# 2gunsu/monocon-pytorch

Measured on AMD Instinct MI355X. Metric: images/sec (384x1280) fwd+bwd, higher is better.
Workload: dtype f32 (f16x2); 1 GPU; train step B=32/GPU 3x384x1280 (configs[2] shape, fp32 values, mode f16x2); global_batch=32, parallelism=dp1, precision_mode=f16x2

## Files before the change

### monocon-pytorch_amd/csrc/kernels_head_train.hip

```cpp
#include <type_traits>

#include "kernels.h"
#include "train.h"

namespace mc {

struct HeadBwdArgs {
    const float *draw; int ld;
    const unsigned *nz; int nz_tiles;
    const float *z, *x, *w1;
    const float *scale, *shift;
    float *d, *dw_partial, *red_partial;
    int HW, rows_per_block, blocks_per_img;
    const float *coef;
    float *csum;
    unsigned *amax;
};
constexpr int HB_PX = 64, HB_LD = 80;
static bool head_rows_as_coded() {
    const int *rbeg = head_row_begin();
    static const int RB[NUM_HEADS + 1] = {0, 3, 5, 7, 25, 34, 36, 39, 41, 65};
    for (int i = 0; i <= NUM_HEADS; ++i)
        if (rbeg[i] != RB[i]) return false;
    return true;
}
__device__ __forceinline__ int head_of_row(int r) {
    return (r >= 3) + (r >= 5) + (r >= 7) + (r >= 25) + (r >= 34) + (r >= 36) + (r >= 39) + (r >= 41);
}
constexpr int HB_WAVES = 4, HB_NT = HB_WAVES * 64, HB_MAXR = 24;

template <int RB, int NR, int MODE>
struct HeadPart {
    static constexpr int CP = NUM_HEADS * HEAD_CH;
    float w[NR], acc[NR];
    float s1, s2, zsc, zsh, cp, cq, cr;
    const float *xp, *zp;
    float *dp;
    bool rez;
    int h, sub, nsub;

    __device__ __forceinline__ void init(const HeadBwdArgs &a, int h_, int lane, size_t p0, int b, int sub_, int nsub_) {
        h = h_; sub = sub_; nsub = nsub_;
#pragma unroll
        for (int r = 0; r < NR; ++r) { w[r] = a.w1[(RB + r) * HEAD_CH + lane]; acc[r] = 0.f; }
        s1 = 0.f; s2 = 0.f;
        rez = a.z == nullptr;
        zsc = rez ? a.scale[(size_t)b * CP + h * HEAD_CH + lane] : 0.f;
        zsh = rez ? a.shift[(size_t)b * CP + h * HEAD_CH + lane] : 0.f;
        xp = a.x + p0 * CP + h * HEAD_CH + lane;
// ... 63 lines not shown
        int k = 0;
        for (; k + U <= cnt; k += U) {
            float xv[U];
#pragma unroll
            for (int u = 0; u < U; ++u) xv[u] = xp[(size_t)(px0 + sub + (k + u) * nsub) * CP];
#pragma unroll
            for (int u = 0; u < U; ++u) {
                const float o = fmaf(cq, xv[u], cr);
                s1 += o;
                s2 = fmaxf(s2, fabsf(o));
                dp[(size_t)(px0 + sub + (k + u) * nsub) * CP] = o;
            }
        }
        for (; k < cnt; ++k) {
            const size_t gp = (size_t)(px0 + sub + k * nsub);
            const float o = fmaf(cq, xp[gp * CP], cr);
            s1 += o;
            s2 = fmaxf(s2, fabsf(o));
            dp[gp * CP] = o;
        }
    }
    __device__ __forceinline__ void spill(float *red, int lane) const {
        if (nsub == 1 || sub == 0) return;
        float *q = red + (size_t)(sub - 1) * (NR + 2) * 64 + lane;
        if (MODE != 2) {
#pragma unroll
            for (int r = 0; r < NR; ++r) q[r * 64] = acc[r];
        }
        q[NR * 64] = s1;
        q[(NR + 1) * 64] = s2;
    }
    __device__ __forceinline__ void finish(const HeadBwdArgs &a, const float *red, int blk, int lane) {
        if (MODE == 2 && a.amax) amax_update_wave(a.amax, s2);
        if (sub != 0) return;
        for (int k = 1; k < nsub; ++k) {
            const float *q = red + (size_t)(k - 1) * (NR + 2) * 64 + lane;
            if (MODE != 2) {
#pragma unroll
                for (int r = 0; r < NR; ++r) acc[r] += q[r * 64];
                s2 += q[(NR + 1) * 64];
            }
            s1 += q[NR * 64];
        }
        if (MODE == 2) {
            a.csum[((size_t)blk * CP + h * HEAD_CH + lane) * 2] = s1;
            return;
        }
#pragma unroll
        for (int r = 0; r < NR; ++r) a.dw_partial[((size_t)blk * NUM_OUT_ROWS + RB + r) * HEAD_CH + lane] = acc[r];
        float *rp = a.red_partial + ((size_t)blk * CP + h * HEAD_CH + lane) * 2;
        rp[0] = s1;
        rp[1] = s2;
    }
};

template <int RB, int NR, int MODE>
__device__ __forceinline__ void head_bwd_one(const HeadBwdArgs &a, float *gsh, float *red, int h, int wv, int lane, size_t p0, int np,
                                             int blk, int b, int r0) {
    HeadPart<RB, NR, MODE> P;
    P.init(a, h, lane, p0, b, wv, HB_WAVES);
    const unsigned *nzb = a.nz ? a.nz + (size_t)b * a.nz_tiles : nullptr;
    auto live = [&](int px0) -> bool {
        if (!nzb) return true;
        const int first = r0 + px0, last = r0 + min(px0 + HB_PX, np) - 1;
        const unsigned m = nzb[first >> 6] | nzb[last >> 6];
        return (__builtin_amdgcn_readfirstlane(m) >> h) & 1u;
// ... 15 lines not shown
        const bool nxt = px0 + HB_PX < np && live(px0 + HB_PX);
        if (cur) {
            __syncthreads();
#pragma unroll
            for (int k = 0; k < NL; ++k) {
                const int e = tid + k * HB_NT;
                if (e < NE) gsh[e] = pre[k];
            }
            __syncthreads();
            if (nxt) fetch(px0 + HB_PX);
            P.block(gsh, px0, min(HB_PX, np - px0));
        } else {
            if (nxt) fetch(px0 + HB_PX);
            P.zero_block(px0, min(HB_PX, np - px0));
        }
        cur = nxt;
    }
    P.spill(red, lane);
    __syncthreads();
    P.finish(a, red, blk, lane);
}
template <int MODE, bool WIDE>
__global__ __launch_bounds__(HB_NT) void head_bwd_kernel(const HeadBwdArgs a) {
    __shared__ float gsh[HB_PX * (WIDE ? HB_MAXR : 3)];
    __shared__ float red[(HB_WAVES - 1) * ((WIDE ? HB_MAXR : 3) + 2) * 64];
    const int lane = threadIdx.x & 63;
    const int wv = __builtin_amdgcn_readfirstlane(threadIdx.x >> 6);
    const int blk = blockIdx.x;
    const int b = blk / a.blocks_per_img, rb = blk % a.blocks_per_img;
    const int r0 = rb * a.rows_per_block;
    const int np = min(a.HW, r0 + a.rows_per_block) - r0;
    const size_t p0 = (size_t)b * a.HW + r0;
    if (WIDE) {
        switch (blockIdx.y) {
            case 0: head_bwd_one<41, 24, MODE>(a, gsh, red, 8, wv, lane, p0, np, blk, b, r0); break;
            case 1: head_bwd_one<7, 18, MODE>(a, gsh, red, 3, wv, lane, p0, np, blk, b, r0); break;
            default: head_bwd_one<25, 9, MODE>(a, gsh, red, 4, wv, lane, p0, np, blk, b, r0); break;
        }
    } else {
        switch (blockIdx.y) {
            case 0: head_bwd_one<0, 3, MODE>(a, gsh, red, 0, wv, lane, p0, np, blk, b, r0); break;
            case 1: head_bwd_one<3, 2, MODE>(a, gsh, red, 1, wv, lane, p0, np, blk, b, r0); break;
            case 2: head_bwd_one<5, 2, MODE>(a, gsh, red, 2, wv, lane, p0, np, blk, b, r0); break;
            case 3: head_bwd_one<34, 2, MODE>(a, gsh, red, 5, wv, lane, p0, np, blk, b, r0); break;
            case 4: head_bwd_one<36, 3, MODE>(a, gsh, red, 6, wv, lane, p0, np, blk, b, r0); break;
            default: head_bwd_one<39, 2, MODE>(a, gsh, red, 7, wv, lane, p0, np, blk, b, r0); break;
        }
    }
}
template <int MODE>
static void head_bwd_launch(const HeadBwdArgs &a, int blocks, hipStream_t st) {
    hipLaunchKernelGGL((head_bwd_kernel<MODE, true>), dim3(blocks, 3), dim3(HB_NT), 0, st, a);
    hipLaunchKernelGGL((head_bwd_kernel<MODE, false>), dim3(blocks, 6), dim3(HB_NT), 0, st, a);
}
static hipError_t head_bwd_args(HeadBwdArgs &a, const float *draw, int ld, const float *z, const float *x, const float *w1, int B,
                                int HW, int blocks, const float *scale, const float *shift, const unsigned *nz) {
    if (!head_rows_as_coded()) return hipErrorInvalidValue;
    if (blocks % B || ld != HB_LD) return hipErrorInvalidValue;
    if (!z && (!scale || !shift)) return hipErrorInvalidValue;
    a = HeadBwdArgs{};
    a.draw = draw; a.ld = ld; a.z = z; a.x = x; a.w1 = w1;
    a.scale = scale; a.shift = shift;
    a.nz = nz; a.nz_tiles = (HW + 63) / 64;
    a.HW = HW; a.blocks_per_img = blocks / B; a.rows_per_block = (HW + a.blocks_per_img - 1) / a.blocks_per_img;
    return hipSuccess;
}
hipError_t launch_head_bwd(const float *draw, int ld, const float *z, const float *x, const float *w1, int B, int HW,
                           int blocks, float *d, float *dw_partial, float *red_partial, hipStream_t st, const float *scale,
                           const float *shift, const unsigned *nz) {
    HeadBwdArgs a;
    hipError_t e = head_bwd_args(a, draw, ld, z, x, w1, B, HW, blocks, scale, shift, nz);
    if (e != hipSuccess) return e;
    a.d = d; a.dw_partial = dw_partial; a.red_partial = red_partial;
    if (d) head_bwd_launch<0>(a, blocks, st);
    else head_bwd_launch<1>(a, blocks, st);
    return hipGetLastError();
}
hipError_t launch_head_dx(const float *draw, int ld, const float *x, const float *w1, const float *coef, int B, int HW, int blocks,
                          float *dx, float *csum, float *csum_out, unsigned *amax, hipStream_t st, const float *scale,
                          const float *shift, const unsigned *nz) {
    if (!coef || !dx || !csum || !csum_out) return hipErrorInvalidValue;
    HeadBwdArgs a;
    hipError_t e = head_bwd_args(a, draw, ld, nullptr, x, w1, B, HW, blocks, scale, shift, nz);
    if (e != hipSuccess) return e;
    a.d = dx; a.coef = coef; a.csum = csum; a.amax = amax;
    head_bwd_launch<2>(a, blocks, st);
    return launch_colsum_final(csum, blocks, NUM_HEADS * HEAD_CH, csum_out, st);
}


struct DpredPackArgs {
    const float *dpred[10];
    int ld, B, HW;
    float *out;
    unsigned *nz;
    int row_pred[NUM_OUT_ROWS], row_ch[NUM_OUT_ROWS], pred_c[10];
};
struct DpredUserArgs : DpredPackArgs {
    const float *grad[10];
    const float *pred[10];
    int row_epi[NUM_OUT_ROWS];
};
__device__ __forceinline__ float pred_act_grad(int epi, float y) {
    if (epi == 1) return (y > 1e-4f && y < 1.f - 1e-4f) ? y * (1.f - y) : 0.f;
    if (epi == 2) {
        const float sig = 1.f / (y + 1.f) - 1e-12f;
        return -sig * (1.f - sig) / ((sig + 1e-12f) * (sig + 1e-12f));
    }
    return 1.f;
}
template <bool USER>
__global__ __launch_bounds__(256) void dpred_pack_kernel(const std::conditional_t<USER, DpredUserArgs, DpredPackArgs> a) {
    __shared__ float t[64][NUM_OUT_ROWS + 2];
    __shared__ const float *rowp[NUM_OUT_ROWS];
    __shared__ const float *rowg[USER ? NUM_OUT_ROWS : 1], *rowy[USER ? NUM_OUT_ROWS : 1];
    __shared__ int rowe[USER ? NUM_OUT_ROWS : 1];
    __shared__ unsigned nzw;
    if (threadIdx.x == 0) nzw = 0u;
    const int tiles = (a.HW + 63) / 64;
// ... 637 lines not shown
```

### monocon-pytorch_amd/csrc/mc_train_plan.hip

```cpp
#include <atomic>
#include <deque>
#include <functional>

#include "mc_internal.h"

using namespace mc;

namespace {

using Fn = std::function<int(mc_handle *, hipStream_t)>;

struct PlanSwitches {
    long long lazy_z;
    long long lazy_min;
    long long lazy_feat;
    long long zbits;
    long long grad_pool;
    long long grad_pool_cool;
    long long head_dx_fuse;
    long long head_zskip;
    long long dgrad_s2_thin;
    long long stem_fuse;
    long long bm_epilogue;
    long long wres_bwd;
    long long dual_stream;
    int side_sync_lo = 0, side_sync_hi = 0;
    bool plan_debug = false;
};
const struct { const char *name; long long PlanSwitches::*field; long long def; } SWITCH_TABLE[] = {
    {"MONOCON_HIP_LAZY_Z", &PlanSwitches::lazy_z, 3},
    {"MONOCON_HIP_LAZY_MIN", &PlanSwitches::lazy_min, 900000},
    {"MONOCON_HIP_LAZY_FEAT", &PlanSwitches::lazy_feat, 0},
    {"MONOCON_HIP_ZBITS", &PlanSwitches::zbits, 1},
    {"MONOCON_HIP_GRAD_POOL", &PlanSwitches::grad_pool, 1},
    {"MONOCON_HIP_GRAD_POOL_COOL", &PlanSwitches::grad_pool_cool, 2},
    {"MONOCON_HIP_HEAD_DX_FUSE", &PlanSwitches::head_dx_fuse, 1},
    {"MONOCON_HIP_HEAD_ZSKIP", &PlanSwitches::head_zskip, 1},
    {"MONOCON_HIP_DGRAD_S2_THIN", &PlanSwitches::dgrad_s2_thin, 1},
    {"MONOCON_HIP_STEM_FUSE", &PlanSwitches::stem_fuse, 1},
    {"MONOCON_HIP_BM_EPILOGUE", &PlanSwitches::bm_epilogue, 1},
    {"MONOCON_HIP_WRES_BWD", &PlanSwitches::wres_bwd, 0},
    {"MONOCON_HIP_DUAL_STREAM", &PlanSwitches::dual_stream, 1},
};
PlanSwitches read_switches() {
    PlanSwitches sw{};
    std::string changed;
    for (const auto &d : SWITCH_TABLE) {
        const char *e = std::getenv(d.name);
        sw.*d.field = e ? std::atoll(e) : d.def;
        if (sw.*d.field != d.def) changed += std::string(" ") + d.name + "=" + std::to_string(sw.*d.field);
    }
    if (const char *e = std::getenv("MONOCON_HIP_SIDE_SYNC")) {
        if (std::sscanf(e, "%d:%d", &sw.side_sync_lo, &sw.side_sync_hi) != 2) sw.side_sync_lo = sw.side_sync_hi = 0;
        if (sw.side_sync_lo < sw.side_sync_hi) changed += std::string(" MONOCON_HIP_SIDE_SYNC=") + e;
    }
    sw.plan_debug = std::getenv("MONOCON_HIP_PLAN_DEBUG") != nullptr;
    if (sw.plan_debug && !changed.empty()) fprintf(stderr, "[plan] switches off their defaults:%s\n", changed.c_str());
    return sw;
}

struct PoolBwdArgs {
    const float *x, *dout, *la, *lb;
    float *dx, *stats;
    int B, H, W, C, acc;
};

struct LastWriter {
    enum Kind { NONE, DGRAD_CONV, POOL_BWD, DECONV_BWD } kind = NONE;
    union {
        ConvPlan *conv;
// ... 597 lines not shown
        { size_t o = 0; for (int i = 0; i < 15; ++i) { tp[i] = ta ? ta + o : nullptr; o += up(tn[i]); } }
        T.center_heatmap_target = tp[0]; T.kpt_heatmap_target = tp[1];
        T.wh_target = tp[2]; T.offset_target = tp[3]; T.dim_target = tp[4];
        T.alpha_cls_target = tp[5]; T.alpha_offset_target = tp[6]; T.depth_target = tp[7];
        T.center2kpt_offset_target = tp[8]; T.kpt_heatmap_offset_target = tp[9];
        T.indices = reinterpret_cast<int64_t *>(tp[10]); T.indices_kpt = reinterpret_cast<int64_t *>(tp[11]);
        T.mask_target = reinterpret_cast<uint8_t *>(tp[12]);
        T.mask_center2kpt_offset = tp[13]; T.mask_kpt_heatmap_offset = tp[14];
        h->tgt_arena = ta; h->tgt_arena_bytes = ttot * sizeof(float);
        ts->dpred[0] = alloc((size_t)B * PRED_CH[0] * HW);
        ts->dpred[1] = alloc((size_t)B * PRED_CH[1] * HW);
        size_t dtot = 0;
        for (int i = 2; i < 10; ++i) dtot += up((size_t)B * PRED_CH[i] * HW);
        float *da = alloc(dtot);
        { size_t o = 0; for (int i = 2; i < 10; ++i) { ts->dpred[i] = da ? da + o : nullptr; o += up((size_t)B * PRED_CH[i] * HW); } }
        h->dp_arena = da; h->dp_arena_bytes = dtot * sizeof(float);
        ts->fwd.push_back([ts = ts, B = B, fh = fh, fw = fw](mc_handle *hh, hipStream_t st) {
            if (mc_make_targets(hh, &ts->labels, B, ts->max_objs, ts->pad_h, ts->pad_w, fh, fw, &ts->targets, st)) return -1;
            if (mc_losses(hh, ts->preds, &ts->targets, B, ts->max_objs, fh, fw, ts->losses, st)) return -1;
            return 0;
        });
    }

    void heads_backward(int feat) {
        float *draw = alloc(raw_numel);
        const size_t nz_words = (size_t)B * ((HW + 63) / 64);
        unsigned *nz = sw.head_zskip ? reinterpret_cast<unsigned *>(alloc(nz_words)) : nullptr;
        const unsigned *nz_bwd = nz, *nz_dx = sw.head_zskip == 1 ? nz : nullptr;
        if (sw.plan_debug)
            fprintf(stderr, "[plan] heads backward: zero-tile skip %s (%zu tile words)\n",
                    !sw.head_zskip ? "off" : sw.head_zskip == 1 ? "on" : "on in the statistics pass only", sw.head_zskip ? nz_words : (size_t)0);
        float *cs1 = alloc(colsum_partial_floats((size_t)B * HW, LD));
        float *db1 = alloc(NUM_OUT_ROWS), *dw1 = alloc((size_t)NUM_OUT_ROWS * HEAD_CH);
        push_bwd([=, ts = ts, B = B, fh = fh, fw = fw, HW = HW](mc_handle *hh, hipStream_t st) {
            if (mc_losses_backward(hh, ts->preds, &ts->targets, B, ts->max_objs, fh, fw, ts->grad_losses, ts->dpred, st)) return -1;
            bool user = false;
            for (const float *g : ts->grad_preds) user = user || g != nullptr;
            if (user)
                HIPCHK(hh, launch_dpred_pack_user(ts->dpred, ts->preds, ts->grad_preds, LD, B, HW, draw, st, nz));
            else
                HIPCHK(hh, launch_dpred_pack(ts->dpred, LD, B, HW, draw, st, nz));
            HIPCHK(hh, launch_colsum(draw, (size_t)B * HW, NUM_OUT_ROWS, LD, cs1, db1, st));
            return 0;
        });
        const int nbr = chan_reduce_blocks(B, HW), rb_per_img = nbr / B;
        const bool dx_fuse = sw.head_dx_fuse != 0;
        float *dh = alloc(xh.numel());
        float *dw1p = alloc((size_t)nbr * NUM_OUT_ROWS * HEAD_CH);
        float *partial = alloc((size_t)nbr * CP * 2), *coef = alloc((size_t)B * CP * 4);
        float *dx = dh;
        CopyBatch segcb;
        auto seg = [&](const std::string &layer, int r0, int nr) {
            if (!segcb.add(dw1 + (size_t)r0 * HEAD_CH, G(layer + ".weight", nr * HEAD_CH), (size_t)nr * HEAD_CH) ||
                !segcb.add(db1 + r0, G(layer + ".bias", nr), nr))
                ts->ok = false;
        };
        for (int hd = 0; hd < NUM_HEADS; ++hd)
            for (const HeadOutLayer &o : mc_head_keys(hd).out) seg(o.layer, o.row0, o.rows);
        const float *xp = xh.p, *w1 = h->head_w1, *zsc = at.scale, *zsh = at.shift;
        push_bwd([=, B = B, HW = HW](mc_handle *hh, hipStream_t st) {
            HIPCHK(hh, launch_head_bwd(draw, LD, nullptr, xp, w1, B, HW, nbr, dx_fuse ? nullptr : dh, dw1p, partial, st, zsc, zsh, nz_bwd));
            HIPCHK(hh, launch_splitk_reduce(dw1p, nbr, 1, NUM_OUT_ROWS, HEAD_CH, dw1, st));
            HIPCHK(hh, launch_copy_batch(segcb, st));
            return 0;
        });
        float *db3 = alloc(CP), *dw3 = alloc((size_t)CP * 64 * 9);
        float *cs3 = alloc((size_t)std::max(affine_bwd_blocks(B, (size_t)HW, CP), nbr) * CP * 2);
        Tensor dxT = xh; dxT.p = dx; dxT.amax = slot();
        unsigned *dxmax = dxT.amax;
        push_bwd([=, at = at, gp = gp, B = B, HW = HW](mc_handle *hh, hipStream_t st) {
            HIPCHK(hh, launch_attn_train_bwd(at, partial, rb_per_img, gp, coef, st));
            if (dx_fuse)
                HIPCHK(hh, launch_head_dx(draw, LD, xp, w1, coef, B, HW, nbr, dx, cs3, db3, dxmax, st, zsc, zsh, nz_dx));
            else
                HIPCHK(hh, launch_affine_bwd(dh, nullptr, xp, coef, B, (size_t)HW, CP, 1, 0, dx, nullptr, 0, st, nullptr, nullptr, cs3, db3,
                                             dxmax));
            return 0;
        });
        emit_wgrad({feat}, dxT, CP, CP, 3, 1, dw3);
        CopyBatch g3cb;
        for (int hd = 0; hd < NUM_HEADS; ++hd) {
            const std::string layer = mc_head_keys(hd).conv3;
            if (!g3cb.add(dw3 + (size_t)hd * 64 * 64 * 9, G(layer + ".weight", 9 * HEAD_CH * HEAD_CH), (size_t)64 * 64 * 9) ||
                !g3cb.add(db3 + hd * 64, G(layer + ".bias", HEAD_CH), 64))
                ts->ok = false;
        }
        push_bwd([=](mc_handle *hh, hipStream_t st) { HIPCHK(hh, launch_copy_batch(g3cb, st)); return 0; }, ON_SIDE);
        CopyBatch w3cb;
        for (int hd = 0; hd < NUM_HEADS; ++hd)
            if (!w3cb.add(P(mc_head_keys(hd).conv3 + ".weight", 9 * HEAD_CH * HEAD_CH), w3dense + (size_t)hd * 64 * 64 * 9,
                          (size_t)64 * 64 * 9))
                ts->ok = false;
        ts->pack_fns.push_back([=](mc_handle *hh, hipStream_t st) { HIPCHK(hh, launch_copy_batch(w3cb, st)); return 0; });
        if (h->prec == 3) h->w_amax_of[w3dense] = h->head3.w_amax;
        emit_dgrad(w3dense, dxT, CP, 64, 3, 1, 0, feat, CP);
        if (ts->head_only) ts->bwd.back().feat_dgrad = true;
    }

    void pool_backward(const Rec &r) {
        TNode &in = ts->nodes[r.in];
        const TNode &o = ts->nodes[r.z];
        if (!o.ginit || !in.needs_grad) return;
        float *gi = g_acquire(r.in);
        PoolBwdArgs pa{in.t.p, o.g, in.t.la, in.t.lb, gi, nullptr, in.t.B, in.t.H, in.t.W, in.t.C, in.ginit ? 1 : 0};
        ts->pool_bwds.push_back(pa);
        PoolBwdArgs *pp = &ts->pool_bwds.back();
        push_bwd([=](mc_handle *hh, hipStream_t st) {
            HIPCHK(hh, launch_maxpool2_bwd(pp->x, pp->dout, pp->B, pp->H, pp->W, pp->C, pp->dx, pp->acc, st, pp->la, pp->lb, pp->stats));
            return 0;
        });
        wrote(r.in, pp);
        g_release(r.z, -1);
    }

    void deconv_backward(const Rec &r) {
        TNode &in = ts->nodes[r.in];
        const TNode &o = ts->nodes[r.z];
        if (!o.ginit) return;
        if (in.ginit) { ts->ok = false; h->err = "train plan: deconv input has more than one consumer"; }
        const float *xp = in.t.p, *go = o.g, *wp = r.D->wpk, *xla = in.t.la, *xlb = in.t.lb;
// ... 397 lines not shown
```

### monocon-pytorch_amd/csrc/train.h

```cpp
#pragma once
#include <hip/hip_runtime.h>
#include <stdint.h>
#include <cstdlib>
#include <vector>

#include "conv_mfma.h"

namespace mc {

struct TargetArgs {
    const float *gt_bboxes, *gt_labels, *gt_bboxes_3d, *depths, *gt_kpts_2d, *gt_kpts_valid, *mask;
    int B, max_objs, num_kpt, num_classes, fh, fw;
    float h_ratio, w_ratio;
    float *center_heatmap, *kpt_heatmap;
    float *wh, *offset, *dim, *alpha_cls, *alpha_offset, *depth, *c2k, *kho;
    long long *indices, *indices_kpt;
    uint8_t *mask_target;
    float *mask_c2k, *mask_kho;
};
hipError_t launch_make_targets(const TargetArgs &a, hipStream_t st);

hipError_t launch_focal(const float *p, const float *t, size_t n, float *partial, float *loss_out, float *aux,
                        hipStream_t st);
hipError_t launch_focal_grad(const float *p, const float *t, size_t n, const float *aux, const float *gscale, int gidx,
// ... 152 lines not shown
                                const float *wpk, float *din,
                                float *stats = nullptr);

hipError_t launch_dpred_pack(const float *const dpred[10], int ld, int B, int HW, float *out, hipStream_t st,
                             unsigned *nz = nullptr);
hipError_t launch_dpred_pack_user(const float *const dpred[10], const float *const pred[10], const float *const grad[10], int ld,
                                  int B, int HW, float *out, hipStream_t st, unsigned *nz = nullptr);
struct AttnTrainArgs {
    const float *stats;
    int chunks, stat_ld, B, HW;
    double *stats64;
    float *rm[9], *rv[9];
    long long *nbt[9];
    const float *att_w[9], *att_g[9], *att_b[9];
    float *att_rm[9], *att_rv[9];
    long long *att_nbt[9];
    const float *weight_[9], *bias_[9];
    float *sv_inst;
    float *mu_r;
    float *bn10;
    float *that, *yatt;
    float *gamma_p;
    float *scale, *shift;
};
struct AttnGradPtrs { float *d_weight_[9], *d_bias_[9], *d_att_w[9], *d_att_g[9], *d_att_b[9]; };
hipError_t launch_attn_train_fwd(const AttnTrainArgs &a, hipStream_t st);
hipError_t launch_attn_train_bwd(const AttnTrainArgs &a, const float *partial, int rb_per_img, const AttnGradPtrs &gp,
                                 float *coef, hipStream_t st);
hipError_t launch_head_bwd(const float *draw, int ld, const float *z, const float *x, const float *w1, int B, int HW,
                           int blocks, float *d, float *dw_partial, float *red_partial, hipStream_t st,
                           const float *scale = nullptr, const float *shift = nullptr, const unsigned *nz = nullptr);
hipError_t launch_head_dx(const float *draw, int ld, const float *x, const float *w1, const float *coef, int B, int HW, int blocks,
                          float *dx, float *csum, float *csum_out, unsigned *amax, hipStream_t st, const float *scale,
                          const float *shift, const unsigned *nz = nullptr);
hipError_t launch_splitk_reduce(const float *partial, int ksplit, int T, int Cout, int Cin, float *dw, hipStream_t st);
int stem_wgrad_blocks(int B, int H, int W);
hipError_t launch_stem_wgrad(const float *img, const float *dy, int B, int H, int W, float *partial, float *dw,
                             hipStream_t st, const unsigned *img_amax = nullptr, const unsigned *dy_amax = nullptr,
                             const float *y = nullptr, const float *coef = nullptr, const unsigned *y_amax = nullptr);
hipError_t launch_stem_dgrad(const float *dy, const float *w_oihw, int B, int H, int W, float *dx, hipStream_t st,
                             const float *y = nullptr, const float *coef = nullptr);

enum WgKernel { WG_FP32, WG_SPLIT, WG_PIPE, WG_SMALL, WG_THIN16 };
struct WgradArgs {
    ConvSrc src[4];
    int nsrc;
    int B, Hin, Win, Hout, Wout, Cin, Cout;
    const float *dy;
    int dy_ld;
    float *partial;
    int ksplit, n_tiles, c_tiles, ppr, ppi, groups_per_img;
    int kernel;
    int prec;
    int pb;
    int pipe;
    const unsigned *amax_x[4], *amax_dy;
};
static_assert(sizeof(WgradArgs) == 264, "WgradArgs is the kernels' parameter block: keep its layout");
struct WgradPlan {
    WgradArgs a;
    int ks, stride;
    int WN, WC;
    bool lazy_ok;
    bool ok;
    size_t partial_floats;
};
inline void wgrad_set_patches(WgradArgs &a, int pb) {
    a.ppr = (a.Wout + 7) / 8;
    a.ppi = a.ppr * ((a.Hout + 3) / 4);
    a.groups_per_img = (a.ppi + pb - 1) / pb;
}
inline bool wgrad_any_lazy(const WgradArgs &a) { return any_lazy_src(a.src, a.nsrc); }
template <int WN_, int WC_>
struct WgTile { static constexpr int WN = WN_, WC = WC_; };
template <typename F>
inline hipError_t with_wgrad_tile(int WN, int WC, F &&f) {
    if (WN == 2 && WC == 2) return f(WgTile<2, 2>{});
    if (WN == 4) return f(WgTile<4, 1>{});
    if (WN == 2) return f(WgTile<2, 1>{});
    return f(WgTile<1, 1>{});
}
inline size_t wgrad_lds_request(size_t need) {
#ifdef MC_DEBUG_HOOKS
    static const size_t pad = [] { const char *e = std::getenv("MONOCON_HIP_WGRAD_LDS_KB"); return e ? (size_t)std::atoi(e) * 1024 : (size_t)0; }();
    return pad > need ? pad : need;
#else
    return need;
#endif
}
void wgrad_plan(WgradPlan &p);
hipError_t launch_wgrad(const WgradPlan &p, float *dw_oihw, hipStream_t st);
inline size_t wgrad_partial_floats(const WgradPlan &p) { return p.partial_floats; }
inline bool wgrad_lazy_capable(const WgradPlan &p) { return p.lazy_ok; }
bool wgrad_is_small(const WgradArgs &a, int ks, int stride);
bool wgrad_thin_ok(const WgradArgs &a, int ks, int stride);
int wgrad_pipe_tile(const WgradArgs &a, int ks, int stride);
void wgrad_shape(const WgradArgs &a, int *WN, int *WC);
bool wgrad_sources_ok(const WgradArgs &a);
bool wgrad_bf16_ok(const WgradArgs &a, int ks, int stride);
hipError_t launch_wgrad_fp32(const WgradPlan &p, hipStream_t st);
hipError_t launch_wgrad_small(const WgradPlan &p, hipStream_t st);
hipError_t launch_wgrad_bf16(const WgradPlan &p, hipStream_t st);
hipError_t launch_wgrad_pipe(const WgradPlan &p, hipStream_t st);
// ... 4 lines not shown
```

### monocon-pytorch_amd/csrc/wgrad_bf16.hip

```cpp
#include "wgrad_tile.h"

namespace mc {

template <int KS, int S, int WN, int WC, int SPL>
struct WgB16Cfg : WgLds<KS, S> {
    static constexpr int PB = SPL == 1 ? 2 : 1;
    static constexpr int NB = 32 * WN, CB = 32 * WC, NT = 64 * WN * WC;
    static constexpr int X_PLANE = PB * CB * WgLds<KS, S>::XCH, D_PLANE = PB * NB * WgLds<KS, S>::DCH;
    static constexpr int X_BYTES = SPL * X_PLANE, D_BYTES = SPL * D_PLANE;
    static constexpr size_t LDS_BYTES = X_BYTES + D_BYTES;
};

template <int KS, int S, int WN, int WC, int SPL, bool LZ = false>
#ifndef MC_WG16_S2_OCC
#define MC_WG16_S2_OCC 1
#endif
__global__ __launch_bounds__(64 * WN * WC, S == 2 ? MC_WG16_S2_OCC : 2) void wgrad_bf16_kernel(const WgradArgs a) {
    using Cfg = WgB16Cfg<KS, S, WN, WC, SPL>;
    typedef typename Piece<SPL>::T pc_t;
    typedef typename Piece<SPL>::V8 pc8;
    typedef typename Piece<SPL>::V2 pc2;
    constexpr int XPL = Cfg::X_PLANE, DPL = Cfg::D_PLANE;
    constexpr int PB = Cfg::PB, NB = Cfg::NB, CB = Cfg::CB, NT = Cfg::NT, PAD = Cfg::PAD;
    constexpr int IH = Cfg::IH, IW = Cfg::IW, XROW = Cfg::XROW, XCH = Cfg::XCH, DCH = Cfg::DCH;
// ... 60 lines not shown
    }
    int d_stat[NID], d_mx[NID], d_dst[NID];
#pragma unroll
    for (int i = 0; i < NID; ++i) {
        const int e = tid + NT * i, item = (e / NC4) % 16;
        const int my = item / 4, mx = (item % 4) * 2;
        d_mx[i] = (dn_ok && e < DP) ? mx : DEAD;
        d_stat[i] = ((my * a.Wout + mx) * a.dy_ld + n0 + dn4 * 4) * 4;
        d_dst[i] = (dn4 * 4) * DCH + lds_skew(dn4 * 4) + my * 16 + mx * 2;
    }

#ifndef MC_WG16_PD
#define MC_WG16_PD 1
#endif
    constexpr int PD = MC_WG16_PD;
    f32x4 xv[PD][PB][NIX][2], dv[PD][PB][NID][2];
    static_assert(!LZ || SPL == 2, "lazy sources: the fp16-split mode");
    const bool lz = LZ && a.src[si].la != nullptr;
    f32x4 lzA = {0.f, 0.f, 0.f, 0.f}, lzB = lzA;
    if (LZ && lz && xc_ok) {
        lzA = *reinterpret_cast<const f32x4 *>(a.src[si].la + cs0 + xc4 * 4);
        lzB = *reinterpret_cast<const f32x4 *>(a.src[si].lb + cs0 + xc4 * 4);
#pragma unroll
        for (int j = 0; j < 4; ++j) { lzA[j] *= x_scale; lzB[j] *= x_scale; }
    }
    [[maybe_unused]] const unsigned x_bytes = (unsigned)(a.Hin * a.Win * Cs) * 4u;
    [[maybe_unused]] unsigned okm[PD][PB];
    auto fetch = [&](int gi, int p, int slot) {
        const int img = __builtin_amdgcn_readfirstlane(gi / a.groups_per_img);
        const int pp = (gi - img * a.groups_per_img) * PB + p;
        const __amdgpu_buffer_rsrc_t r_x =
            make_rsrc(xsrc + (size_t)img * a.Hin * a.Win * Cs, (unsigned)(a.Hin * a.Win * Cs) * 4u);
        const __amdgpu_buffer_rsrc_t r_d =
            make_rsrc(a.dy + (size_t)img * a.Hout * a.Wout * a.dy_ld, (unsigned)(a.Hout * a.Wout * a.dy_ld) * 4u);
        const bool valid = pp < a.ppi;
        const int prow = __builtin_amdgcn_readfirstlane(pp / a.ppr);
        const int oy = prow * 4, ox = valid ? (pp - prow * a.ppr) * 8 : DEAD;
        const int xb = (oy * S * a.Win + ox * S) * Cs * 4;
        const int db = (oy * a.Wout + ox) * a.dy_ld * 4;
        if constexpr (LZ) okm[slot][p] = 0u;
#pragma unroll
        for (int i = 0; i < NIX; ++i) {
            const int xx = ox * S + x_ix[i];
            const bool in0 = wg_in_row(xx, a.Win), in1 = wg_in_row(xx + S, a.Win);
            const int vo0 = in0 ? xb + x_stat[i] : BUF_OOB, vo1 = in1 ? xb + x_stat[i] + S * Cs * 4 : BUF_OOB;
            xv[slot][p][i][0] = buf_load4(r_x, vo0, 0);
            xv[slot][p][i][1] = buf_load4(r_x, vo1, 0);
            if constexpr (LZ) okm[slot][p] |= (((unsigned)vo0 < x_bytes ? 1u : 0u) | ((unsigned)vo1 < x_bytes ? 2u : 0u)) << (2 * i);
        }
#pragma unroll
        for (int i = 0; i < NID; ++i) {
            const int xx = ox + d_mx[i];
            const bool in0 = wg_in_row(xx, a.Wout), in1 = wg_in_row(xx + 1, a.Wout);
            dv[slot][p][i][0] = buf_load4(r_d, in0 ? db + d_stat[i] : BUF_OOB, 0);
            dv[slot][p][i][1] = buf_load4(r_d, in1 ? db + d_stat[i] + a.dy_ld * 4 : BUF_OOB, 0);
        }
    };
    auto put = [&](unsigned char *dst, int plane, f32x4 v0, f32x4 v1, int chan_stride, float scale) {
#pragma unroll
        for (int j = 0; j < 4; ++j) {
            float r0 = SPL == 2 ? v0[j] * scale : v0[j], r1 = SPL == 2 ? v1[j] * scale : v1[j];
#pragma unroll
            for (int q = 0; q < SPL; ++q) {
                pc2 pr;
                pr[0] = (pc_t)r0;
                pr[1] = (pc_t)r1;
                *reinterpret_cast<unsigned *>(dst + q * plane + j * chan_stride) = __builtin_bit_cast(unsigned, pr);
// ... 144 lines not shown
```

### monocon-pytorch_amd/csrc/wgrad_mfma.hip

```cpp
#include "conv_mfma.h"
#include "train.h"

namespace mc {

template <int KS, int S, int WN, int WC>
struct WgCfg {
    static constexpr int PB = 2;
    static constexpr int NB = 32 * WN, CB = 32 * WC;
    static constexpr int NT = 64 * WN * WC;
    static constexpr int PAD = KS / 2;
    static constexpr int IH = 3 * S + KS, IW = 7 * S + KS, NPIX = IH * IW;
    static constexpr int CBP = CB + 4, NBP = NB + 4;
    static constexpr int LDS_FLOATS = PB * NPIX * CBP + PB * 32 * NBP;
    static constexpr size_t LDS_BYTES = sizeof(float) * LDS_FLOATS;
};

template <int KS, int S, int WN, int WC>
__global__ __launch_bounds__(64 * WN * WC, 2) void wgrad_mfma_kernel(const WgradArgs a) {
    using Cfg = WgCfg<KS, S, WN, WC>;
    constexpr int PB = Cfg::PB, NB = Cfg::NB, CB = Cfg::CB, NT = Cfg::NT, PAD = Cfg::PAD;
    constexpr int IW = Cfg::IW, NPIX = Cfg::NPIX, CBP = Cfg::CBP, NBP = Cfg::NBP;
    constexpr int T = KS * KS;
    extern __shared__ __attribute__((aligned(16))) float lds[];
    float *xt = lds;
// ... 26 lines not shown
    constexpr int XC4 = CB / 4, XP = NPIX * XC4, NIX = (XP + NT - 1) / NT;
    constexpr int NC4 = NB / 4, DP = 32 * NC4, NID = (DP + NT - 1) / NT;
    static_assert(NT % XC4 == 0 && NT % NC4 == 0, "static channel group per thread");
    constexpr int DEAD = -(1 << 24);
    const int xc4 = tid % XC4, dn4 = tid % NC4;
    const bool xc_ok = cs0 + xc4 * 4 < Cs && c0 + xc4 * 4 < a.Cin;
    const bool dn_ok = n0 + dn4 * 4 + 3 < a.dy_ld;
    int x_stat[NIX], x_ix[NIX];
#pragma unroll
    for (int i = 0; i < NIX; ++i) {
        const int e = tid + NT * i, pix = (e / XC4) % NPIX;
        const int iy = pix / IW, ix = pix % IW;
        x_ix[i] = (xc_ok && e < XP) ? ix - PAD : DEAD;
        x_stat[i] = (((iy - PAD) * a.Win + ix - PAD) * Cs + cs0 + xc4 * 4) * 4;
    }
    int d_stat[NID], d_mx[NID];
#pragma unroll
    for (int i = 0; i < NID; ++i) {
        const int e = tid + NT * i, m = (e / NC4) % 32;
        d_mx[i] = (dn_ok && e < DP) ? (m & 7) : -DEAD;
        d_stat[i] = (((m >> 3) * a.Wout + (m & 7)) * a.dy_ld + n0 + dn4 * 4) * 4;
    }
    float *x_dst = xt + (tid / XC4) * CBP + xc4 * 4;
    float *d_dst = dyt + (tid / NC4) * NBP + dn4 * 4;

    f32x4 xv[PB][NIX], dv[PB][NID];
    constexpr bool PF = S == 1 && NT >= 128;
    auto fetch = [&](int gi, int p) {
        const int img = gi / a.groups_per_img;
        const int pp = (gi - img * a.groups_per_img) * PB + p;
        const __amdgpu_buffer_rsrc_t r_x =
            make_rsrc(xsrc + (size_t)img * a.Hin * a.Win * Cs, (unsigned)(a.Hin * a.Win * Cs) * 4u);
        const __amdgpu_buffer_rsrc_t r_d =
            make_rsrc(a.dy + (size_t)img * a.Hout * a.Wout * a.dy_ld, (unsigned)(a.Hout * a.Wout * a.dy_ld) * 4u);
        const bool valid = pp < a.ppi;
        const int oy = (pp / a.ppr) * 4, ox = valid ? (pp % a.ppr) * 8 : DEAD;
        const int xb = ((oy * S) * a.Win + ox * S) * Cs * 4;
        const int db = (oy * a.Wout + ox) * a.dy_ld * 4;
#pragma unroll
        for (int i = 0; i < NIX; ++i) {
            const int xx = ox * S + x_ix[i];
            xv[PF ? p : 0][i] = buf_load4(r_x, (xx >= 0 && xx < a.Win) ? xb + x_stat[i] : BUF_OOB, 0);
        }
#pragma unroll
        for (int i = 0; i < NID; ++i) {
            const int xx = ox + d_mx[i];
            dv[PF ? p : 0][i] = buf_load4(r_d, (xx >= 0 && xx < a.Wout) ? db + d_stat[i] : BUF_OOB, 0);
        }
    };
    auto store = [&](int p) {
#pragma unroll
        for (int i = 0; i < NIX; ++i)
            if (NT * (i + 1) <= XP || tid + NT * i < XP)
                *reinterpret_cast<f32x4 *>(x_dst + (p * NPIX + i * (NT / XC4)) * CBP) = xv[PF ? p : 0][i];
#pragma unroll
        for (int i = 0; i < NID; ++i)
            if (NT * (i + 1) <= DP || tid + NT * i < DP)
                *reinterpret_cast<f32x4 *>(d_dst + (p * 32 + i * (NT / NC4)) * NBP) = dv[PF ? p : 0][i];
    };

    const float *a_base = dyt + g * NBP + wn * 32 + li;
    const float *b_base = xt + (g * S) * CBP + wc * 32 + li;

    if (PF && g_begin < g_end) {
#pragma unroll
        for (int p = 0; p < PB; ++p) fetch(g_begin, p);
    }
// ... 255 lines not shown
```

### monocon-pytorch_amd/csrc/wgrad_pipe.hip

```cpp
#include <cstdlib>
#include "wgrad_tile.h"

namespace mc {

template <int V> struct WpInt { static constexpr int value = V; };

template <int KS, int WN, int WC, int WK>
struct WgPipeCfg : WgLds<KS, 1> {
    static constexpr int NB = 32 * WN, CB = 32 * WC, NW = WN * WC * WK, NT = 64 * NW;
    static constexpr int X_PLANE = CB * WgLds<KS, 1>::XCH, D_PLANE = NB * WgLds<KS, 1>::DCH;
    static constexpr int BUF = 2 * (X_PLANE + D_PLANE);
    static constexpr size_t LDS_BYTES = 2 * BUF;
    static_assert(LDS_BYTES <= 160 * 1024, "two tile buffers per CU");
};

__device__ __forceinline__ void wp_barrier() { asm volatile("s_waitcnt lgkmcnt(0)\n\ts_barrier" ::: "memory"); }

template <int KS, int WN, int WC, int WK, bool LZ = false>
__global__ __launch_bounds__(64 * WN * WC * WK, WN * WC * WK == 4 ? 2 : 1) void wgrad_pipe_kernel(const WgradArgs a) {
    using Cfg = WgPipeCfg<KS, WN, WC, WK>;
    constexpr int NB = Cfg::NB, CB = Cfg::CB, NT = Cfg::NT, PAD = Cfg::PAD, IH = Cfg::IH, IW = Cfg::IW, T = Cfg::T;
    constexpr int XROW = Cfg::XROW, XCH = Cfg::XCH, DCH = Cfg::DCH, XPL = Cfg::X_PLANE, DPL = Cfg::D_PLANE, BUF = Cfg::BUF;
    extern __shared__ __attribute__((aligned(16))) unsigned char lds_raw[];

// ... 50 lines not shown
        const int e0 = tid + NT * i, e = e0 < DP ? e0 : e0 - KD, item = (e / NC4) % 16;
        const int my = item / 4, mx = (item % 4) * 2;
        d_mx[i] = dn_ok ? mx : DEAD;
        d_stat[i] = ((my * a.Wout + mx) * a.dy_ld + n0 + dn4 * 4) * 4;
        d_dst[i] = 2 * XPL + (dn4 * 4) * DCH + lds_skew(dn4 * 4) + my * 16 + mx * 2;
    }

    f32x4 xv[2][NIX][2], dv[2][NID][2];
    const bool lz = LZ && a.src[si].la != nullptr;
    [[maybe_unused]] f32x4 *lz_tab = reinterpret_cast<f32x4 *>(lds_raw + 2 * BUF);
    if constexpr (LZ) {
        if (lz && tid < XC4) {
            f32x4 cA = {0.f, 0.f, 0.f, 0.f}, cB = cA;
            if (cs0 + tid * 4 < Cs && c0 + tid * 4 < a.Cin) {
                cA = *reinterpret_cast<const f32x4 *>(a.src[si].la + cs0 + tid * 4);
                cB = *reinterpret_cast<const f32x4 *>(a.src[si].lb + cs0 + tid * 4);
            }
#pragma unroll
            for (int j = 0; j < 4; ++j) { cA[j] *= x_scale; cB[j] *= x_scale; }
            lz_tab[tid] = cA;
            lz_tab[XC4 + tid] = cB;
        }
        __syncthreads();
    }
    [[maybe_unused]] const unsigned x_bytes = (unsigned)(a.Hin * a.Win * Cs) * 4u;
    [[maybe_unused]] unsigned okm[2] = {0u, 0u};
    auto fetch = [&](int gi, auto slot_c) {
        constexpr int slot = decltype(slot_c)::value;
        const int img = __builtin_amdgcn_readfirstlane(gi / a.groups_per_img);
        const int pp = gi - img * a.groups_per_img;
        const __amdgpu_buffer_rsrc_t r_x =
            make_rsrc(xsrc + (size_t)img * a.Hin * a.Win * Cs, (unsigned)(a.Hin * a.Win * Cs) * 4u);
        const __amdgpu_buffer_rsrc_t r_d =
            make_rsrc(a.dy + (size_t)img * a.Hout * a.Wout * a.dy_ld, (unsigned)(a.Hout * a.Wout * a.dy_ld) * 4u);
        const int prow = __builtin_amdgcn_readfirstlane(pp / a.ppr);
        const int oy = prow * 4, ox = (pp - prow * a.ppr) * 8;
        const int xb = (oy * a.Win + ox) * Cs * 4;
        const int db = (oy * a.Wout + ox) * a.dy_ld * 4;
        if constexpr (LZ) okm[slot] = 0u;
#pragma unroll
        for (int i = 0; i < NIX; ++i) {
            const int xx = ox + x_ix[i];
            const bool in0 = wg_in_row(xx, a.Win), in1 = wg_in_row(xx + 1, a.Win);
            const int vo0 = in0 ? xb + x_stat[i] : BUF_OOB, vo1 = in1 ? xb + x_stat[i] + Cs * 4 : BUF_OOB;
            xv[slot][i][0] = buf_load4(r_x, vo0, 0);
            xv[slot][i][1] = buf_load4(r_x, vo1, 0);
            if constexpr (LZ) okm[slot] |= (((unsigned)vo0 < x_bytes ? 1u : 0u) | ((unsigned)vo1 < x_bytes ? 2u : 0u)) << (2 * i);
        }
#pragma unroll
        for (int i = 0; i < NID; ++i) {
            const int xx = ox + d_mx[i];
            const bool in0 = wg_in_row(xx, a.Wout), in1 = wg_in_row(xx + 1, a.Wout);
            dv[slot][i][0] = buf_load4(r_d, in0 ? db + d_stat[i] : BUF_OOB, 0);
            dv[slot][i][1] = buf_load4(r_d, in1 ? db + d_stat[i] + a.dy_ld * 4 : BUF_OOB, 0);
        }
    };
    auto put = [&](unsigned char *dst, int plane, const f32x4 v0, const f32x4 v1, int chan_stride, float scale) {
#pragma unroll
        for (int j = 0; j < 4; ++j) {
            unsigned hi, lo;
            split_pair(v0[j], v1[j], scale, hi, lo);
            *reinterpret_cast<unsigned *>(dst + j * chan_stride) = hi;
            *reinterpret_cast<unsigned *>(dst + plane + j * chan_stride) = lo;
        }
    };
    auto store_x = [&](unsigned char *buf, auto slot_c, int i) {
        constexpr int slot = decltype(slot_c)::value;
// ... 133 lines not shown
```

Baseline: 694.8 images/sec.

## Split head dx and 3x3 weight gradient into pipelined head groups

Adds an optional mode that computes the fused head dx pass per group of heads and launches each group's 3x3 weight gradient as soon as that slice is ready, so the weight gradient overlaps the remaining dx work. It also moves small reductions (bias colsums, split-k reduce, gradient copies, final colsum for the 3x3 bias) to the side stream when dx fusion is on. The wgrad kernels' dy buffer bound is tightened so that channel slices of dx can be read safely. The grouped mode is off by default and adds extra launches and per-group amax slots.

Result: no change. 697.1 images/sec, median of 5 (+0.3%).

```diff
diff --git a/monocon-pytorch_amd/csrc/kernels_head_train.hip b/monocon-pytorch_amd/csrc/kernels_head_train.hip
--- a/monocon-pytorch_amd/csrc/kernels_head_train.hip
+++ b/monocon-pytorch_amd/csrc/kernels_head_train.hip
@@ -1,3 +1,4 @@
+#include <algorithm>
 #include <type_traits>
 
 #include "kernels.h"
@@ -15,6 +16,8 @@
     const float *coef;
     float *csum;
     unsigned *amax;
+    int y0;
+    unsigned *amax_grp;
 };
 constexpr int HB_PX = 64, HB_LD = 80;
 static bool head_rows_as_coded() {
@@ -144,6 +147,7 @@
     }
     __device__ __forceinline__ void finish(const HeadBwdArgs &a, const float *red, int blk, int lane) {
         if (MODE == 2 && a.amax) amax_update_wave(a.amax, s2);
+        if (MODE == 2 && a.amax_grp) amax_update_wave(a.amax_grp, s2);
         if (sub != 0) return;
         for (int k = 1; k < nsub; ++k) {
             const float *q = red + (size_t)(k - 1) * (NR + 2) * 64 + lane;
@@ -225,13 +229,13 @@
     const int np = min(a.HW, r0 + a.rows_per_block) - r0;
     const size_t p0 = (size_t)b * a.HW + r0;
     if (WIDE) {
-        switch (blockIdx.y) {
+        switch (blockIdx.y + a.y0) {
             case 0: head_bwd_one<41, 24, MODE>(a, gsh, red, 8, wv, lane, p0, np, blk, b, r0); break;
             case 1: head_bwd_one<7, 18, MODE>(a, gsh, red, 3, wv, lane, p0, np, blk, b, r0); break;
             default: head_bwd_one<25, 9, MODE>(a, gsh, red, 4, wv, lane, p0, np, blk, b, r0); break;
         }
     } else {
-        switch (blockIdx.y) {
+        switch (blockIdx.y + a.y0) {
             case 0: head_bwd_one<0, 3, MODE>(a, gsh, red, 0, wv, lane, p0, np, blk, b, r0); break;
             case 1: head_bwd_one<3, 2, MODE>(a, gsh, red, 1, wv, lane, p0, np, blk, b, r0); break;
             case 2: head_bwd_one<5, 2, MODE>(a, gsh, red, 2, wv, lane, p0, np, blk, b, r0); break;
@@ -269,15 +273,33 @@
     else head_bwd_launch<1>(a, blocks, st);
     return hipGetLastError();
 }
+static const int WIDE_Y[NUM_HEADS] = {-1, -1, -1, 1, 2, -1, -1, -1, 0}, NARROW_Y[NUM_HEADS] = {0, 1, 2, -1, -1, 3, 4, 5, -1};
 hipError_t launch_head_dx(const float *draw, int ld, const float *x, const float *w1, const float *coef, int B, int HW, int blocks,
                           float *dx, float *csum, float *csum_out, unsigned *amax, hipStream_t st, const float *scale,
-                          const float *shift, const unsigned *nz) {
-    if (!coef || !dx || !csum || !csum_out) return hipErrorInvalidValue;
+                          const float *shift, const unsigned *nz, int head0, int nheads, unsigned *amax_grp) {
+    if (!coef || !dx || !csum) return hipErrorInvalidValue;
+    if (head0 < 0 || nheads < 1 || head0 + nheads > NUM_HEADS) return hipErrorInvalidValue;
+    if (csum_out && nheads != NUM_HEADS) return hipErrorInvalidValue;
     HeadBwdArgs a;
     hipError_t e = head_bwd_args(a, draw, ld, nullptr, x, w1, B, HW, blocks, scale, shift, nz);
     if (e != hipSuccess) return e;
-    a.d = dx; a.coef = coef; a.csum = csum; a.amax = amax;
-    head_bwd_launch<2>(a, blocks, st);
+    a.d = dx; a.coef = coef; a.csum = csum; a.amax = amax; a.amax_grp = amax_grp;
+    int lo[2] = {NUM_HEADS, NUM_HEADS}, hi[2] = {-1, -1}, cnt[2] = {0, 0};
+    for (int h = head0; h < head0 + nheads; ++h) {
+        const int k = WIDE_Y[h] >= 0 ? 0 : 1, y = k ? NARROW_Y[h] : WIDE_Y[h];
+        lo[k] = std::min(lo[k], y); hi[k] = std::max(hi[k], y); ++cnt[k];
+    }
+    for (int k = 0; k < 2; ++k)
+        if (cnt[k] && hi[k] - lo[k] + 1 != cnt[k]) return hipErrorInvalidValue;
+    if (cnt[0]) {
+        a.y0 = lo[0];
+        hipLaunchKernelGGL((head_bwd_kernel<2, true>), dim3(blocks, cnt[0]), dim3(HB_NT), 0, st, a);
+    }
+    if (cnt[1]) {
+        a.y0 = lo[1];
+        hipLaunchKernelGGL((head_bwd_kernel<2, false>), dim3(blocks, cnt[1]), dim3(HB_NT), 0, st, a);
+    }
+    if (!csum_out) return hipGetLastError();
     return launch_colsum_final(csum, blocks, NUM_HEADS * HEAD_CH, csum_out, st);
 }
 
diff --git a/monocon-pytorch_amd/csrc/mc_train_plan.hip b/monocon-pytorch_amd/csrc/mc_train_plan.hip
--- a/monocon-pytorch_amd/csrc/mc_train_plan.hip
+++ b/monocon-pytorch_amd/csrc/mc_train_plan.hip
@@ -19,6 +19,7 @@
     long long grad_pool_cool;
     long long head_dx_fuse;
     long long head_zskip;
+    long long head_pipe;
     long long dgrad_s2_thin;
     long long stem_fuse;
     long long bm_epilogue;
@@ -36,6 +37,7 @@
     {"MONOCON_HIP_GRAD_POOL_COOL", &PlanSwitches::grad_pool_cool, 2},
     {"MONOCON_HIP_HEAD_DX_FUSE", &PlanSwitches::head_dx_fuse, 1},
     {"MONOCON_HIP_HEAD_ZSKIP", &PlanSwitches::head_zskip, 1},
+    {"MONOCON_HIP_HEAD_PIPE", &PlanSwitches::head_pipe, 0},
     {"MONOCON_HIP_DGRAD_S2_THIN", &PlanSwitches::dgrad_s2_thin, 1},
     {"MONOCON_HIP_STEM_FUSE", &PlanSwitches::stem_fuse, 1},
     {"MONOCON_HIP_BM_EPILOGUE", &PlanSwitches::bm_epilogue, 1},
@@ -699,6 +701,19 @@
                     !sw.head_zskip ? "off" : sw.head_zskip == 1 ? "on" : "on in the statistics pass only", sw.head_zskip ? nz_words : (size_t)0);
         float *cs1 = alloc(colsum_partial_floats((size_t)B * HW, LD));
         float *db1 = alloc(NUM_OUT_ROWS), *dw1 = alloc((size_t)NUM_OUT_ROWS * HEAD_CH);
+        const bool dx_fuse = sw.head_dx_fuse != 0;
+        const BwdStream small = dx_fuse ? ON_SIDE : ON_MAIN;
+        const int ngroups = (dx_fuse && (sw.head_pipe == 3 || sw.head_pipe == 9)) ? (int)sw.head_pipe : 0;
+        if (sw.plan_debug) {
+            std::string gs;
+            for (int g = 0; g < ngroups; ++g) {
+                gs += " {";
+                for (int k = 0; k < NUM_HEADS / ngroups; ++k) gs += (k ? "," : "") + std::to_string(g * (NUM_HEADS / ngroups) + k);
+                gs += "}";
+            }
+            if (ngroups) fprintf(stderr, "[plan] heads backward: dx pass and 3x3 weight gradient in %d head groups%s\n", ngroups, gs.c_str());
+            else fprintf(stderr, "[plan] heads backward: weight gradient per head group off\n");
+        }
         push_bwd([=, ts = ts, B = B, fh = fh, fw = fw, HW = HW](mc_handle *hh, hipStream_t st) {
             if (mc_losses_backward(hh, ts->preds, &ts->targets, B, ts->max_objs, fh, fw, ts->grad_losses, ts->dpred, st)) return -1;
             bool user = false;
@@ -707,11 +722,15 @@
                 HIPCHK(hh, launch_dpred_pack_user(ts->dpred, ts->preds, ts->grad_preds, LD, B, HW, draw, st, nz));
             else
                 HIPCHK(hh, launch_dpred_pack(ts->dpred, LD, B, HW, draw, st, nz));
-            HIPCHK(hh, launch_colsum(draw, (size_t)B * HW, NUM_OUT_ROWS, LD, cs1, db1, st));
-            return 0;
-        });
+            if (small == ON_MAIN) HIPCHK(hh, launch_colsum(draw, (size_t)B * HW, NUM_OUT_ROWS, LD, cs1, db1, st));
+            return 0;
+        });
+        if (small == ON_SIDE)
+            push_bwd([=, B = B, HW = HW](mc_handle *hh, hipStream_t st) {
+                HIPCHK(hh, launch_colsum(draw, (size_t)B * HW, NUM_OUT_ROWS, LD, cs1, db1, st));
+                return 0;
+            }, ON_SIDE);
         const int nbr = chan_reduce_blocks(B, HW), rb_per_img = nbr / B;
-        const bool dx_fuse = sw.head_dx_fuse != 0;
         float *dh = alloc(xh.numel());
         float *dw1p = alloc((size_t)nbr * NUM_OUT_ROWS * HEAD_CH);
         float *partial = alloc((size_t)nbr * CP * 2), *coef = alloc((size_t)B * CP * 4);
@@ -727,24 +746,51 @@
         const float *xp = xh.p, *w1 = h->head_w1, *zsc = at.scale, *zsh = at.shift;
         push_bwd([=, B = B, HW = HW](mc_handle *hh, hipStream_t st) {
             HIPCHK(hh, launch_head_bwd(draw, LD, nullptr, xp, w1, B, HW, nbr, dx_fuse ? nullptr : dh, dw1p, partial, st, zsc, zsh, nz_bwd));
-            HIPCHK(hh, launch_splitk_reduce(dw1p, nbr, 1, NUM_OUT_ROWS, HEAD_CH, dw1, st));
-            HIPCHK(hh, launch_copy_batch(segcb, st));
-            return 0;
-        });
+            if (small == ON_MAIN) {
+                HIPCHK(hh, launch_splitk_reduce(dw1p, nbr, 1, NUM_OUT_ROWS, HEAD_CH, dw1, st));
+                HIPCHK(hh, launch_copy_batch(segcb, st));
+            }
+            return 0;
+        });
+        if (small == ON_SIDE)
+            push_bwd([=](mc_handle *hh, hipStream_t st) {
+                HIPCHK(hh, launch_splitk_reduce(dw1p, nbr, 1, NUM_OUT_ROWS, HEAD_CH, dw1, st));
+                HIPCHK(hh, launch_copy_batch(segcb, st));
+                return 0;
+            }, ON_SIDE);
         float *db3 = alloc(CP), *dw3 = alloc((size_t)CP * 64 * 9);
         float *cs3 = alloc((size_t)std::max(affine_bwd_blocks(B, (size_t)HW, CP), nbr) * CP * 2);
         Tensor dxT = xh; dxT.p = dx; dxT.amax = slot();
         unsigned *dxmax = dxT.amax;
+        const int per = ngroups ? NUM_HEADS / ngroups : NUM_HEADS;
+        unsigned *gmax0 = ngroups ? slot() : nullptr;
         push_bwd([=, at = at, gp = gp, B = B, HW = HW](mc_handle *hh, hipStream_t st) {
             HIPCHK(hh, launch_attn_train_bwd(at, partial, rb_per_img, gp, coef, st));
             if (dx_fuse)
-                HIPCHK(hh, launch_head_dx(draw, LD, xp, w1, coef, B, HW, nbr, dx, cs3, db3, dxmax, st, zsc, zsh, nz_dx));
+                HIPCHK(hh, launch_head_dx(draw, LD, xp, w1, coef, B, HW, nbr, dx, cs3, nullptr, dxmax, st, zsc, zsh, nz_dx, 0, per, gmax0));
             else
                 HIPCHK(hh, launch_affine_bwd(dh, nullptr, xp, coef, B, (size_t)HW, CP, 1, 0, dx, nullptr, 0, st, nullptr, nullptr, cs3, db3,
                                              dxmax));
             return 0;
         });
-        emit_wgrad({feat}, dxT, CP, CP, 3, 1, dw3);
+        if (!ngroups) {
+            emit_wgrad({feat}, dxT, CP, CP, 3, 1, dw3);
+        } else {
+            auto group_wgrad = [&](int g, unsigned *gmax) {
+                Tensor dyg = dxT;
+                dyg.p = dx + (size_t)g * per * HEAD_CH; dyg.amax = gmax;
+                emit_wgrad({feat}, dyg, CP, per * HEAD_CH, 3, 1, dw3 + (size_t)g * per * HEAD_CH * 64 * 9);
+            };
+            group_wgrad(0, gmax0);
+            for (int g = 1; g < ngroups; ++g) {
+                unsigned *gmax = slot();
+                push_bwd([=, B = B, HW = HW](mc_handle *hh, hipStream_t st) {
+                    HIPCHK(hh, launch_head_dx(draw, LD, xp, w1, coef, B, HW, nbr, dx, cs3, nullptr, dxmax, st, zsc, zsh, nz_dx, g * per, per, gmax));
+                    return 0;
+                });
+                group_wgrad(g, gmax);
+            }
+        }
         CopyBatch g3cb;
         for (int hd = 0; hd < NUM_HEADS; ++hd) {
             const std::string layer = mc_head_keys(hd).conv3;
@@ -752,7 +798,11 @@
                 !g3cb.add(db3 + hd * 64, G(layer + ".bias", HEAD_CH), 64))
                 ts->ok = false;
         }
-        push_bwd([=](mc_handle *hh, hipStream_t st) { HIPCHK(hh, launch_copy_batch(g3cb, st)); return 0; }, ON_SIDE);
+        push_bwd([=](mc_handle *hh, hipStream_t st) {
+            if (dx_fuse) HIPCHK(hh, launch_colsum_final(cs3, nbr, CP, db3, st));
+            HIPCHK(hh, launch_copy_batch(g3cb, st));
+            return 0;
+        }, ON_SIDE);
         CopyBatch w3cb;
         for (int hd = 0; hd < NUM_HEADS; ++hd)
             if (!w3cb.add(P(mc_head_keys(hd).conv3 + ".weight", 9 * HEAD_CH * HEAD_CH), w3dense + (size_t)hd * 64 * 64 * 9,
diff --git a/monocon-pytorch_amd/csrc/train.h b/monocon-pytorch_amd/csrc/train.h
--- a/monocon-pytorch_amd/csrc/train.h
+++ b/monocon-pytorch_amd/csrc/train.h
@@ -208,7 +208,8 @@
                            const float *scale = nullptr, const float *shift = nullptr, const unsigned *nz = nullptr);
 hipError_t launch_head_dx(const float *draw, int ld, const float *x, const float *w1, const float *coef, int B, int HW, int blocks,
                           float *dx, float *csum, float *csum_out, unsigned *amax, hipStream_t st, const float *scale,
-                          const float *shift, const unsigned *nz = nullptr);
+                          const float *shift, const unsigned *nz = nullptr,
+                          int head0 = 0, int nheads = 9, unsigned *amax_grp = nullptr);
 hipError_t launch_splitk_reduce(const float *partial, int ksplit, int T, int Cout, int Cin, float *dw, hipStream_t st);
 int stem_wgrad_blocks(int B, int H, int W);
 hipError_t launch_stem_wgrad(const float *img, const float *dy, int B, int H, int W, float *partial, float *dw,
@@ -245,6 +246,9 @@
     a.ppr = (a.Wout + 7) / 8;
     a.ppi = a.ppr * ((a.Hout + 3) / 4);
     a.groups_per_img = (a.ppi + pb - 1) / pb;
+}
+__host__ __device__ __forceinline__ unsigned wg_dy_bytes(const WgradArgs &a) {
+    return (unsigned)((a.Hout * a.Wout - 1) * a.dy_ld + a.Cout) * 4u;
 }
 inline bool wgrad_any_lazy(const WgradArgs &a) { return any_lazy_src(a.src, a.nsrc); }
 template <int WN_, int WC_>
diff --git a/monocon-pytorch_amd/csrc/wgrad_bf16.hip b/monocon-pytorch_amd/csrc/wgrad_bf16.hip
--- a/monocon-pytorch_amd/csrc/wgrad_bf16.hip
+++ b/monocon-pytorch_amd/csrc/wgrad_bf16.hip
@@ -116,7 +116,7 @@
         const __amdgpu_buffer_rsrc_t r_x =
             make_rsrc(xsrc + (size_t)img * a.Hin * a.Win * Cs, (unsigned)(a.Hin * a.Win * Cs) * 4u);
         const __amdgpu_buffer_rsrc_t r_d =
-            make_rsrc(a.dy + (size_t)img * a.Hout * a.Wout * a.dy_ld, (unsigned)(a.Hout * a.Wout * a.dy_ld) * 4u);
+            make_rsrc(a.dy + (size_t)img * a.Hout * a.Wout * a.dy_ld, wg_dy_bytes(a));
         const bool valid = pp < a.ppi;
         const int prow = __builtin_amdgcn_readfirstlane(pp / a.ppr);
         const int oy = prow * 4, ox = valid ? (pp - prow * a.ppr) * 8 : DEAD;
diff --git a/monocon-pytorch_amd/csrc/wgrad_mfma.hip b/monocon-pytorch_amd/csrc/wgrad_mfma.hip
--- a/monocon-pytorch_amd/csrc/wgrad_mfma.hip
+++ b/monocon-pytorch_amd/csrc/wgrad_mfma.hip
@@ -82,7 +82,7 @@
         const __amdgpu_buffer_rsrc_t r_x =
             make_rsrc(xsrc + (size_t)img * a.Hin * a.Win * Cs, (unsigned)(a.Hin * a.Win * Cs) * 4u);
         const __amdgpu_buffer_rsrc_t r_d =
-            make_rsrc(a.dy + (size_t)img * a.Hout * a.Wout * a.dy_ld, (unsigned)(a.Hout * a.Wout * a.dy_ld) * 4u);
+            make_rsrc(a.dy + (size_t)img * a.Hout * a.Wout * a.dy_ld, wg_dy_bytes(a));
         const bool valid = pp < a.ppi;
         const int oy = (pp / a.ppr) * 4, ox = valid ? (pp % a.ppr) * 8 : DEAD;
         const int xb = ((oy * S) * a.Win + ox * S) * Cs * 4;
diff --git a/monocon-pytorch_amd/csrc/wgrad_pipe.hip b/monocon-pytorch_amd/csrc/wgrad_pipe.hip
--- a/monocon-pytorch_amd/csrc/wgrad_pipe.hip
+++ b/monocon-pytorch_amd/csrc/wgrad_pipe.hip
@@ -106,7 +106,7 @@
         const __amdgpu_buffer_rsrc_t r_x =
             make_rsrc(xsrc + (size_t)img * a.Hin * a.Win * Cs, (unsigned)(a.Hin * a.Win * Cs) * 4u);
         const __amdgpu_buffer_rsrc_t r_d =
-            make_rsrc(a.dy + (size_t)img * a.Hout * a.Wout * a.dy_ld, (unsigned)(a.Hout * a.Wout * a.dy_ld) * 4u);
+            make_rsrc(a.dy + (size_t)img * a.Hout * a.Wout * a.dy_ld, wg_dy_bytes(a));
         const int prow = __builtin_amdgcn_readfirstlane(pp / a.ppr);
         const int oy = prow * 4, ox = (pp - prow * a.ppr) * 8;
         const int xb = (oy * a.Win + ox) * Cs * 4;
```
